# tkortz/opencv

Hardware: AMD Instinct MI355X
Metric: tracked frames/sec, 1080p×128-object TBD loop @ 1/2/4/8 MI355X (higher is better)
Workload: dtype u8; 1 GPU; TBD loop 1920x1080 x 128 objects (BASELINE configs[2]), frames [5, 2577) of a 2577-frame sequence per GPU; levels=3, win=21, gftt=256/box, q 0.01, minDist 3, every 5, tracker_bounds=reference, parallelism=replicas x1 (one sequence per GPU), api=tbdk_tbd_run (native frame loop, look-ahead)

## Files before the change

### opencv_amd/csrc/klt_lk_multi.hip

```cpp
#include <type_traits>

#include "lk_device.hpp"

namespace tbdk {

namespace {

using namespace lkdev;

__device__ __forceinline__ uint32_t scan64(uint32_t v)
{
    v += (uint32_t)__builtin_amdgcn_update_dpp(0, (int)v, 0x111, 0xF, 0xF, true);
    v += (uint32_t)__builtin_amdgcn_update_dpp(0, (int)v, 0x112, 0xF, 0xF, true);
    v += (uint32_t)__builtin_amdgcn_update_dpp(0, (int)v, 0x114, 0xF, 0xF, true);
    v += (uint32_t)__builtin_amdgcn_update_dpp(0, (int)v, 0x118, 0xF, 0xF, true);
    v += (uint32_t)__builtin_amdgcn_update_dpp(0, (int)v, 0x142, 0xA, 0xF, false);
    v += (uint32_t)__builtin_amdgcn_update_dpp(0, (int)v, 0x143, 0xC, 0xF, false);
    return v;
}

template <int M>
__device__ __forceinline__ void scan64_n(uint32_t (&v)[M])
{
#define TBDK_SCAN_STEP(ctrl, rmask, bc)                                                                    \
    _Pragma("unroll") for (int m = 0; m < M; ++m) v[m] +=                                                  \
        (uint32_t)__builtin_amdgcn_update_dpp(0, (int)v[m], ctrl, rmask, 0xF, bc);
    TBDK_SCAN_STEP(0x111, 0xF, true)
    TBDK_SCAN_STEP(0x112, 0xF, true)
    TBDK_SCAN_STEP(0x114, 0xF, true)
    TBDK_SCAN_STEP(0x118, 0xF, true)
    TBDK_SCAN_STEP(0x142, 0xA, false)
    TBDK_SCAN_STEP(0x143, 0xC, false)
#undef TBDK_SCAN_STEP
}

__device__ __forceinline__ uint32_t seg_total(uint32_t scanned, int e4, int s4)
{
    return (uint32_t)__builtin_amdgcn_ds_bpermute(e4, (int)scanned) -
           (uint32_t)__builtin_amdgcn_ds_bpermute(s4, (int)scanned);
}

template <int N, int FB = 26>
__device__ __forceinline__ void seg_sum_exact(const int (&v)[N], int e4, int s4, float (&out)[N], bool* split = nullptr)
{
    static_assert(N >= 1 && N <= 3, "three 11-bit fields per packed scan");
    static_assert(FB <= 26, "hi parts are v >> 26");
    bool big = false;
#pragma unroll
    for (int k = 0; k < N; ++k) big |= (uint32_t)v[k] + (1u << FB) >= (2u << FB);
    const bool slow = __builtin_amdgcn_ballot_w64(big) != 0;
    if (split) *split = slow;
    if (!slow) {
        uint32_t sv[N];
#pragma unroll
        for (int k = 0; k < N; ++k) sv[k] = (uint32_t)v[k];
        scan64_n(sv);
#pragma unroll
        for (int k = 0; k < N; ++k) out[k] = (float)(int)seg_total(sv[k], e4, s4);
        return;
    }
    uint32_t sc[N + 1];
    sc[N] = 0;
#pragma unroll
    for (int k = 0; k < N; ++k) {
        sc[k] = (uint32_t)v[k] & 0x3FFFFFFu;
        sc[N] += (uint32_t)(v[k] >> 26) << (11 * k);
    }
    scan64_n(sc);
    int h = (int)seg_total(sc[N], e4, s4);
#pragma unroll
    for (int k = 0; k < N; ++k) {
        const int hk = k + 1 < N ? (int)((uint32_t)h << 21) >> 21 : h;
        h = (h - hk) >> 11;
        const uint32_t l = seg_total(sc[k], e4, s4);
        out[k] = (float)((double)hk * 67108864.0 + (double)l);
    }
}

__device__ __forceinline__ int seg_sum_small(int v, int e4, int s4)
{
    return (int)seg_total(scan64((uint32_t)v), e4, s4);
}

__device__ __forceinline__ int bilin_c(uint32_t p0, uint32_t p1, uint32_t w0, uint32_t w1, int c)
{
    int t;
    asm("v_dot2_i32_i16 %0, %1, %2, %3" : "=v"(t) : "v"(p1), "v"(w1), "v"(c));
    return sdot2(p0, w0, t);
}

template <int SH>
__device__ __forceinline__ uint32_t pack_shr(int t0, int t1)
{
    uint32_t d = (uint32_t)(t0 >> SH);
    asm("v_ashrrev_i32_sdwa %0, %2, %1 dst_sel:WORD_1 dst_unused:UNUSED_PRESERVE src0_sel:DWORD src1_sel:DWORD"
        : "+v"(d)
        : "v"(t1), "i"(SH));
    return d;
}
__device__ __forceinline__ uint32_t pack_diff(int t0, int t1) { return pack_shr<9>(t0, t1); }

__device__ __forceinline__ bool any_lane(bool p) { return __builtin_amdgcn_ballot_w64(p) != 0; }


}

#ifndef TBDK_LK_IPACK
#define TBDK_LK_IPACK 1
#endif
#ifndef TBDK_LK_IPACK_FLY
#define TBDK_LK_IPACK_FLY 0
#endif

#ifdef TBDK_LK_TRACE
__device__ unsigned long long* g_lk_trace;
__device__ unsigned int g_lk_trace_cap;
static unsigned g_lk_trace_next;
#endif

template <int WW, int WH, bool FLY, bool DENSE = false>
__global__ __launch_bounds__(64) void lk_multi_kernel(LkArgs a)
{
    constexpr bool BACK = false;
    const LkBack bk{};
#include "klt_lk_multi_body.inc"
}

template <int WW, int WH>
__global__ __launch_bounds__(64) void lk_multi_back_kernel(LkArgs a, LkBack bk)
{
    constexpr bool BACK = true, FLY = true, DENSE = false;
#include "klt_lk_multi_body.inc"
}

#define TBDK_MULTI_WINDOWS(X) X(7) X(9) X(11) X(13) X(15) X(17) X(19) X(21) X(23) X(25) X(27) X(29) X(31)

bool lk_multi_supported(int win_w, int win_h)
{
    if (win_w != win_h) return false;
    switch (win_w) {
#define TBDK_CASE(W) case W:
        TBDK_MULTI_WINDOWS(TBDK_CASE)
#undef TBDK_CASE
        return true;
    default:
        return false;
    }
}

hipError_t launch_lk_multi(const LkArgs& a, bool fly, hipStream_t s)
{
    if (!lk_multi_supported(a.win_w, a.win_h)) return hipErrorNotSupported;
    const int per_wg = 64 / a.win_w;
    const dim3 grid((a.n + per_wg - 1) / per_wg), block(64);
#ifdef TBDK_LK_TRACE
    LkArgs at = a;
    at.trace_base = g_lk_trace_next;
    g_lk_trace_next += grid.x;
    const LkArgs& la = at;
#else
    const LkArgs& la = a;
#endif
    switch (a.win_w) {
#define TBDK_CASE(W)                                                                    \
    case W:                                                                             \
        if (fly) hipLaunchKernelGGL((lk_multi_kernel<W, W, true>), grid, block, 0, s, la);  \
        else hipLaunchKernelGGL((lk_multi_kernel<W, W, false>), grid, block, 0, s, la); \
        break;
        TBDK_MULTI_WINDOWS(TBDK_CASE)
#undef TBDK_CASE
    default:
        return hipErrorNotSupported;
    }
    return hipGetLastError();
}

hipError_t launch_lk_multi_back(const LkArgs& a, const LkBack& b, hipStream_t s)
{
    if (!lk_multi_supported(a.win_w, a.win_h)) return hipErrorNotSupported;
    const int per_wg = 64 / a.win_w;
    const dim3 grid((a.n + per_wg - 1) / per_wg), block(64);
#ifdef TBDK_LK_TRACE
    LkArgs at = a;
    at.trace_base = g_lk_trace_next;
    g_lk_trace_next += grid.x;
    const LkArgs& la = at;
#else
    const LkArgs& la = a;
#endif
    switch (a.win_w) {
#define TBDK_CASE(W)                                                              \
    case W:                                                                       \
        hipLaunchKernelGGL((lk_multi_back_kernel<W, W>), grid, block, 0, s, la, b); \
        break;
        TBDK_MULTI_WINDOWS(TBDK_CASE)
#undef TBDK_CASE
    default:
        return hipErrorNotSupported;
    }
    return hipGetLastError();
}

hipError_t launch_lk_multi_dense(const LkArgs& a, hipStream_t s)
{
    if (!lk_multi_supported(a.win_w, a.win_h)) return hipErrorNotSupported;
    const int per_wg = 64 / a.win_w;
    const dim3 grid((a.n + per_wg - 1) / per_wg), block(64);
    switch (a.win_w) {
#define TBDK_CASE(W)                                                                          \
    case W:                                                                                   \
        hipLaunchKernelGGL((lk_multi_kernel<W, W, false, true>), grid, block, 0, s, a);       \
        break;
        TBDK_MULTI_WINDOWS(TBDK_CASE)
#undef TBDK_CASE
    default:
        return hipErrorNotSupported;
    }
    return hipGetLastError();
}

}

#ifdef TBDK_LK_TRACE
extern "C" int tbdk_probe_lk_trace(void* buf, unsigned cap)
{
    unsigned long long* p = static_cast<unsigned long long*>(buf);
    cap /= 16;
    if (hipDeviceSynchronize() != hipSuccess ||
        hipMemcpyToSymbol(HIP_SYMBOL(tbdk::g_lk_trace), &p, sizeof(p)) != hipSuccess ||
        hipMemcpyToSymbol(HIP_SYMBOL(tbdk::g_lk_trace_cap), &cap, sizeof(cap)) != hipSuccess)
        return -2;
    tbdk::g_lk_trace_next = 0;
    return 0;
}
extern "C" int tbdk_probe_lk_trace_count(unsigned* n)
{
    *n = tbdk::g_lk_trace_next;
    return 0;
}
#endif
```

### opencv_amd/csrc/klt_lk_multi_body.inc

```
    static_assert(!DENSE || (!FLY && TBDK_LK_IPACK == 1), "dense mode: the planes instance's packed I pairs");
    static_assert(!BACK || (FLY && !DENSE), "backward mode: the Scharr-on-the-fly instance");
    constexpr int P = 64 / WW;
    constexpr int NP = (WH + 1) / 2;
    constexpr int IM = FLY ? TBDK_LK_IPACK_FLY : TBDK_LK_IPACK;
    constexpr bool IPACK = IM == 1, ILIN = IM == 2;
    constexpr bool kSoloOk = P >= 2 && !ILIN;
    const int lane = threadIdx.x & 63;
    const int k = lane == 0 ? P : (lane - 1) / WW;
    const int x = k < P ? lane - 1 - k * WW : 0;
    const int wave = xcd_swizzle(blockIdx.x, gridDim.x) + (threadIdx.x >> 6);
#ifdef TBDK_LK_TRACE
    const unsigned long long tr_t0 = __builtin_amdgcn_s_memrealtime();
#endif
    int i = -1;
    float p0x = 0.f, p0y = 0.f;
    float o0x = 0.f, o0y = 0.f;
    int fst = 0;
    if constexpr (DENSE) {
        i = k < P && wave * P + k < a.n ? wave * P + k : -1;
    } else {
        const int kk = wave * P + k;
        if (k < P && kk < a.n) {
            if (!a.seg_counts) {
                i = kk;
                p0x = a.prev_pts[2 * i];
                p0y = a.prev_pts[2 * i + 1];
                if constexpr (BACK) {
                    o0x = p0x;
                    o0y = p0y;
                    p0x = a.next_pts[2 * i];
                    p0y = a.next_pts[2 * i + 1];
                    fst = a.status[i];
                }
            } else {
                const int seg = kk / a.seg_stride, j = kk - seg * a.seg_stride;
                const int s = a.seg_ninl > 0 ? (int)a.seg_inl[seg] : a.seg_list ? a.seg_list[seg] : seg;
                const int cand = s * a.seg_stride + j;
                const int cnt = a.seg_counts[s];
                const float cx = a.prev_pts[2 * cand], cy = a.prev_pts[2 * cand + 1];
                float nx = 0.f, ny = 0.f;
                int cs = 0;
                if constexpr (BACK) {
                    nx = a.next_pts[2 * cand];
                    ny = a.next_pts[2 * cand + 1];
                    cs = a.status[cand];
                }
                if (j < cnt) {
                    i = cand;
                    p0x = cx;
                    p0y = cy;
                    if constexpr (BACK) {
                        o0x = cx;
                        o0y = cy;
                        p0x = nx;
                        p0y = ny;
                        fst = cs;
                    }
                }
            }
        }
    }
    if constexpr (BACK) {
        if (i >= 0 && !fst) {
            if (x == 0) {
                if (bk.back_pts) {
                    bk.back_pts[2 * i] = o0x;
                    bk.back_pts[2 * i + 1] = o0y;
                }
                if (bk.fb_err) bk.fb_err[i] = __builtin_inff();
            }
            i = -1;
        }
    }
    const bool valid = i >= 0;
    if (!any_lane(valid)) return;
#ifdef TBDK_LK_TRACE
    int tr_steps = 0, tr_reloads = 0;
    unsigned tr_gsplit = 0;
    auto tr_stamp = [&](int idx) {
        const unsigned r = a.trace_base + (unsigned)wave;
        const unsigned d = (unsigned)(__builtin_amdgcn_s_memrealtime() - tr_t0);
        if (lane == 0 && r < g_lk_trace_cap) reinterpret_cast<unsigned*>(g_lk_trace + 16ull * r + 6)[idx] = d;
    };
#else
    auto tr_stamp = [](int) {};
#endif
#ifdef TBDK_LK_TRACE
    asm volatile("s_waitcnt vmcnt(0)" ::: "memory");
    tr_stamp(13);
#endif
    const int e4 = 4 * (k * WW + WW), s4 = 4 * (k * WW);
    const int rnd9 = __builtin_amdgcn_readfirstlane(1 << (W_BITS1 - 5 - 1));
    const int rnd14 = __builtin_amdgcn_readfirstlane(1 << (W_BITS1 - 1));

    const float FLT_SCALE = 1.f / (1 << 20);
    const float halfx = (WW - 1) * 0.5f, halfy = (WH - 1) * 0.5f;
    const int gy = DENSE && valid ? i / a.dense_w : 0, gx = DENSE && valid ? i - gy * a.dense_w : 0;
    if constexpr (DENSE) {
        p0x = (float)gx;
        p0y = (float)gy;
    }
    float outx = 0.f, outy = 0.f;
    if (((BACK ? 0 : a.flags) & TBDK_OPTFLOW_USE_INITIAL_FLOW) && valid) {
        outx = a.next_pts[2 * i];
        outy = a.next_pts[2 * i + 1];
    }
    int status = 1, nit = 0;
#if defined(TBDK_LK_PROBE_RELOADS) && TBDK_LK_PROBE_RELOADS == 2
    int nrl = 0;
#endif
    float errv = 0.f;

    for (int level = a.max_level; level >= 0; --level) {
        const LkLevel L = a.lv[level];
        tr_stamp(4 * level);
        const float sc = (float)(1. / (1 << level));
        float prevx = p0x * sc, prevy = p0y * sc;
        float nextx, nexty;
        if (level == a.max_level) {
            if ((BACK ? 0 : a.flags) & TBDK_OPTFLOW_USE_INITIAL_FLOW) {
                nextx = outx * sc;
                nexty = outy * sc;
            } else {
                nextx = prevx;
                nexty = prevy;
            }
        } else {
            nextx = outx * 2.f;
            nexty = outy * 2.f;
        }
        outx = nextx;
        outy = nexty;

        prevx -= halfx;
        prevy -= halfy;
        const int ipx = (int)floorf(prevx), ipy = (int)floorf(prevy);
        bool act = valid;
        if (ipx < -WW || ipx >= L.w || ipy < -WH || ipy >= L.h) {
            if (level == 0) {
                status = 0;
                errv = 0.f;
            }
            act = false;
        }
        if (!any_lane(act)) continue;
        uint32_t w0, w1;
        bilinear_weights(prevx - ipx, prevy - ipy, w0, w1);

        uint32_t jp[WH + 1];
        const int hp = L.h + 2 * L.ipad;
        const __amdgpu_buffer_rsrc_t rI = make_rsrc(L.I, rsrc_bytes(L.ipitch, hp, L.ipad ? 256 : 0));
        const __amdgpu_buffer_rsrc_t rD = make_rsrc(L.D, rsrc_bytes(L.dpitch, L.h + 2 * L.dpad, 256));
        const __amdgpu_buffer_rsrc_t rJ = make_rsrc(L.J, rsrc_bytes(L.jpitch, L.h + 2 * L.jpad, L.jpad ? 256 : 0));
        auto load_j = [&](bool on, int jx0, int jy0) {
            if (L.jpad == 0 &&
                any_lane(on && (jx0 + x < 0 || jx0 + x + 1 >= L.w || jy0 < 0 || jy0 + WH >= L.h))) {
#pragma unroll
                for (int r = 0; r <= WH; ++r)
                    jp[r] = on ? load_pair_refl(rJ, L.jpitch, L.w, L.h, jy0 + r, jx0 + x) : 0u;
                return;
            }
            const uint32_t joff = on ? (uint32_t)(jy0 + L.jpad) * (uint32_t)L.jpitch + (uint32_t)(jx0 + x + L.jpad) : 0u;
#pragma unroll
            for (int r = 0; r <= WH; ++r) jp[r] = load_pair_u8_ua(rJ, joff, (int)((uint32_t)r * (uint32_t)L.jpitch));
        };

        nextx -= halfx;
        nexty -= halfy;
        int pinx = (int)floorf(nextx), piny = (int)floorf(nexty);

        uint32_t ipk[IPACK ? NP : 1];
        int ic[IM == 0 ? WH : 1];
        int cgx = 0, cgy = 0;
        uint32_t gxk[NP], gyk[NP];
        float A11, A12, A22;
        {
            int acc[3] = {0, 0, 0};
            auto pair_step = [&](int q, uint32_t ip0, uint32_t ip1, uint32_t ip2, uint32_t dx0, uint32_t dx1,
                                 uint32_t dx2, uint32_t dy0, uint32_t dy1, uint32_t dy2, uint32_t dw0, uint32_t dw1,
                                 uint32_t dw2, uint32_t dw3) {
                const int r = 2 * q;
                const bool two = r + 1 < WH;
                uint32_t ipq = 0;
                if constexpr (IPACK || ILIN) {
                    const int i0 = bilin_s<0>(ip0, ip1, w0, w1, rnd9);
                    const int i1 = two ? bilin_s<0>(ip1, ip2, w0, w1, rnd9) : 0;
                    ipq = pack_shr<W_BITS1 - 5>(i0, i1);
                    if constexpr (IPACK) ipk[q] = ipq;
                } else {
                    ic[r] = rnd9 - (bilin_s<W_BITS1 - 5>(ip0, ip1, w0, w1, rnd9) << 9);
                    if (two) ic[r + 1] = rnd9 - (bilin_s<W_BITS1 - 5>(ip1, ip2, w0, w1, rnd9) << 9);
                }
                const int x0 = bilin_s<0>(dx0, dx1, dw0, dw1, rnd14);
                const int x1 = two ? bilin_s<0>(dx1, dx2, dw2, dw3, rnd14) : 0;
                const int y0 = bilin_s<0>(dy0, dy1, dw0, dw1, rnd14);
                const int y1 = two ? bilin_s<0>(dy1, dy2, dw2, dw3, rnd14) : 0;
                gxk[q] = pack_shr<W_BITS1>(x0, x1);
                gyk[q] = pack_shr<W_BITS1>(y0, y1);
                if constexpr (ILIN) {
                    cgx = sdot2(ipq, gxk[q], cgx);
                    cgy = sdot2(ipq, gyk[q], cgy);
                }
                acc[0] = sdot2(gxk[q], gxk[q], acc[0]);
                acc[1] = sdot2(gxk[q], gyk[q], acc[1]);
                acc[2] = sdot2(gyk[q], gyk[q], acc[2]);
            };
            if constexpr (FLY) {
                const uint32_t ioff =
                    act ? (uint32_t)(ipy - 1 + L.ipad) * (uint32_t)L.ipitch + (uint32_t)(ipx + x - 1 + L.ipad) : 0u;
                uint32_t u[WH + 3];
                if (L.ipad == 0 &&
                    any_lane(act && (ipx + x - 1 < 0 || ipx + x + 2 >= L.w || ipy - 1 < 0 || ipy + WH + 1 >= L.h))) {
#pragma unroll
                    for (int r = 0; r < WH + 3; ++r)
                        u[r] = act ? load4_refl(rI, L.ipitch, L.w, L.h, ipy - 1 + r, ipx + x - 1) : 0u;
                } else {
#pragma unroll
                    for (int r = 0; r < WH + 3; ++r)
                        u[r] = __builtin_amdgcn_raw_buffer_load_b32(rI, ioff, (int)((uint32_t)r * (uint32_t)L.ipitch), 0);
                }
#ifdef TBDK_LK_TRACE
                asm volatile("s_waitcnt vmcnt(0)" ::: "memory");
                if (level == a.max_level) tr_stamp(14);
#endif
                const uint32_t cm = ((unsigned)(ipx + x) < (unsigned)L.w ? 0x0000FFFFu : 0u) |
                                    ((unsigned)(ipx + x + 1) < (unsigned)L.w ? 0xFFFF0000u : 0u);
                const int rlo = min(max(-ipy, 0), 32), rhi = min(max(L.h - ipy, 0), 32);
                const uint32_t vm = (uint32_t)(((1ull << rhi) - 1ull) & ~((1ull << rlo) - 1ull));
                const uint32_t wd0 = w0 & cm, wd1 = w1 & cm;
                auto rowbit = [&](int r) { return (uint32_t)((int)(vm << (31 - r)) >> 31); };
                auto src = [&](int j, uint32_t& mid, uint32_t& hd, uint32_t& sm) {
                    const u16x2 lo = as_u16x2(__builtin_amdgcn_perm(0u, u[j], 0x0C010C00u));
                    const u16x2 hi = as_u16x2(__builtin_amdgcn_perm(0u, u[j], 0x0C030C02u));
                    mid = __builtin_amdgcn_perm(0u, u[j], 0x0C020C01u);
                    hd = as_u32(hi - lo);
                    sm = as_u32((lo + hi) * (unsigned short)3 + as_u16x2(mid) * (unsigned short)10);
                };
                auto drow = [&](uint32_t hda, uint32_t hdb, uint32_t hdc, uint32_t sma, uint32_t smc, uint32_t& dx,
                                uint32_t& dy) {
                    dx = as_u32((as_u16x2(hda) + as_u16x2(hdc)) * (unsigned short)3 + as_u16x2(hdb) * (unsigned short)10);
                    dy = as_u32(as_u16x2(smc) - as_u16x2(sma));
                };
                uint32_t m0, h0, s0, m1, h1, s1, m2, h2, s2;
                src(0, m0, h0, s0);
                src(1, m1, h1, s1);
                src(2, m2, h2, s2);
                uint32_t dxa, dya;
                drow(h0, h1, h2, s0, s2, dxa, dya);
                uint32_t ipa = m1;
                uint32_t ra = rowbit(0);
#pragma unroll
                for (int q = 0; q < NP; ++q) {
                    const int r = 2 * q;
                    m0 = m1; h0 = h1; s0 = s1;
                    m1 = m2; h1 = h2; s1 = s2;
                    src(r + 3, m2, h2, s2);
                    uint32_t dxb, dyb, dxc = 0, dyc = 0, ipc = 0;
                    drow(h0, h1, h2, s0, s2, dxb, dyb);
                    const uint32_t ipb = m1;
                    const uint32_t rb = rowbit(r + 1);
                    uint32_t rc = 0;
                    if (r + 1 < WH) {
                        m0 = m1; h0 = h1; s0 = s1;
                        m1 = m2; h1 = h2; s1 = s2;
                        src(r + 4, m2, h2, s2);
                        drow(h0, h1, h2, s0, s2, dxc, dyc);
                        ipc = m1;
                        rc = rowbit(r + 2);
                    }
                    pair_step(q, ipa, ipb, ipc, dxa, dxb, dxc, dya, dyb, dyc, wd0 & ra, wd1 & rb, wd0 & rb, wd1 & rc);
                    ipa = ipc;
                    dxa = dxc;
                    dya = dyc;
                    ra = rc;
                }
            } else if constexpr (DENSE) {
                const int msk = (1 << level) - 1;
                const int64_t cbase = act ? (int64_t)(((gy & msk) << level) | (gx & msk)) * L.cstride +
                                                (int64_t)ipy * L.cpitch + ipx + x
                                          : -(int64_t)(WH / 2) * L.cpitch - WW / 2;
                const uint2* cw = L.C + cbase;
#pragma unroll
                for (int q = 0; q < NP; ++q) {
                    const int r = 2 * q;
                    const uint2 e0 = cw[(int64_t)r * L.cpitch];
                    const uint2 e1 = r + 1 < WH ? cw[(int64_t)(r + 1) * L.cpitch] : make_uint2(0u, 0u);
                    ipk[q] = __builtin_amdgcn_perm(e1.x, e0.x, 0x05040100u);
                    gxk[q] = __builtin_amdgcn_perm(e1.x, e0.x, 0x07060302u);
                    gyk[q] = __builtin_amdgcn_perm(e1.y, e0.y, 0x05040100u);
                    acc[0] = sdot2(gxk[q], gxk[q], acc[0]);
                    acc[1] = sdot2(gxk[q], gyk[q], acc[1]);
                    acc[2] = sdot2(gyk[q], gyk[q], acc[2]);
                }
            } else {
                uint32_t ip[WH + 1], dxp[WH + 1], dyp[WH + 1];
                const uint32_t ioff = act ? (uint32_t)((ipy + L.ipad) * L.ipitch + ipx + x + L.ipad) : 0u;
                const uint32_t doff = act ? (uint32_t)((ipy + L.dpad) * L.dpitch + (ipx + x + L.dpad) * 4) : 0u;
#pragma unroll
                for (int r = 0; r <= WH; ++r) {
                    ip[r] = load_pair_u8_ua(rI, ioff, r * L.ipitch);
                    const uint32_t d0 = __builtin_amdgcn_raw_buffer_load_b32(rD, doff, r * L.dpitch, 0);
                    const uint32_t d1 = __builtin_amdgcn_raw_buffer_load_b32(rD, doff + 4, r * L.dpitch, 0);
                    dxp[r] = __builtin_amdgcn_perm(d1, d0, 0x05040100u);
                    dyp[r] = __builtin_amdgcn_perm(d1, d0, 0x07060302u);
                }
#pragma unroll
                for (int q = 0; q < NP; ++q) {
                    const int r = 2 * q;
                    const int r2 = r + 2 <= WH ? r + 2 : WH;
                    pair_step(q, ip[r], ip[r + 1], ip[r2], dxp[r], dxp[r + 1], dxp[r2], dyp[r], dyp[r + 1], dyp[r2],
                              w0, w1, w0, w1);
                }
            }
            if constexpr (IPACK) {
#pragma unroll
                for (int q = 0; q < NP; ++q) asm volatile("" : "+v"(ipk[q]));
            }
#ifdef TBDK_LK_TRACE
            __builtin_amdgcn_sched_barrier(0);
            if (level == a.max_level) tr_stamp(15);
            __builtin_amdgcn_sched_barrier(0);
#endif
            if (k >= P) acc[0] = acc[1] = acc[2] = 0;
            float s[3];
#ifdef TBDK_LK_TRACE
            bool tr_split = false;
            seg_sum_exact<3>(acc, e4, s4, s, &tr_split);
            tr_gsplit |= tr_split ? 1u << level : 0u;
#else
            seg_sum_exact<3>(acc, e4, s4, s);
#endif
            tr_stamp(4 * level + 1);
            {
                const bool jin = act && !(pinx < -WW || pinx >= L.w || piny < -WH || piny >= L.h);
                load_j(jin, pinx, piny);
#ifdef TBDK_LK_TRACE
                asm volatile("s_waitcnt vmcnt(0)" ::: "memory");
#endif
                tr_stamp(4 * level + 2);
            }
            A11 = s[0] * FLT_SCALE;
            A12 = s[1] * FLT_SCALE;
            A22 = s[2] * FLT_SCALE;
        }
        float D = A11 * A22 - A12 * A12;
        const float minEig =
            (A22 + A11 - sqrtf((A11 - A22) * (A11 - A22) + 4.f * A12 * A12)) / (float)(2 * WW * WH);
        if (act && ((BACK ? 0 : a.flags) & TBDK_OPTFLOW_LK_GET_MIN_EIGENVALS)) errv = minEig;
        if (act && (minEig < a.min_eig || D < 1.19209290e-07F )) {
            if (level == 0) status = 0;
            act = false;
        }
        D = 1.f / D;

        float pdx = 0.f, pdy = 0.f;
        auto solo_steps = [&](int ks, int j) {
            constexpr int NPG = (NP + P - 1) / P;
            constexpr int RG = 2 * NPG;
            const int sl = 1 + ks * WW;
            const int src = k < P ? 4 * (sl + x) : 0;
            const int g = k < P ? k : 0;
            uint32_t gx2[NPG], gy2[NPG], ip2[IPACK ? NPG : 1];
            int ic2[IM == 0 ? RG : 1];
#pragma unroll
            for (int t = 0; t < NPG; ++t) gx2[t] = gy2[t] = 0u;
            if constexpr (IPACK) {
#pragma unroll
                for (int t = 0; t < NPG; ++t) ip2[t] = 0u;
            }
            if constexpr (IM == 0) {
#pragma unroll
                for (int t = 0; t < RG; ++t) ic2[t] = 0;
            }
#pragma unroll
            for (int q = 0; q < NP; ++q) {
                const uint32_t tx = (uint32_t)__builtin_amdgcn_ds_bpermute(src, (int)gxk[q]);
                const uint32_t ty = (uint32_t)__builtin_amdgcn_ds_bpermute(src, (int)gyk[q]);
                gx2[q % NPG] = g == q / NPG ? tx : gx2[q % NPG];
                gy2[q % NPG] = g == q / NPG ? ty : gy2[q % NPG];
                if constexpr (IPACK) {
                    const uint32_t ti = (uint32_t)__builtin_amdgcn_ds_bpermute(src, (int)ipk[q]);
                    ip2[q % NPG] = g == q / NPG ? ti : ip2[q % NPG];
                }
            }
            if constexpr (IM == 0) {
#pragma unroll
                for (int r = 0; r < WH; ++r) {
                    const int ti = __builtin_amdgcn_ds_bpermute(src, ic[r]);
                    ic2[r % RG] = g == r / RG ? ti : ic2[r % RG];
                }
            }
            if (k >= P) {
#pragma unroll
                for (int t = 0; t < NPG; ++t) gx2[t] = gy2[t] = 0u;
            }
            auto bc = [&](float v) { return __int_as_float(__builtin_amdgcn_readlane(__float_as_int(v), sl)); };
            float snx = bc(nextx), sny = bc(nexty), sox = bc(outx), soy = bc(outy), spdx = bc(pdx), spdy = bc(pdy);
            const float sA11 = bc(A11), sA12 = bc(A12), sA22 = bc(A22), sD = bc(D);
            const int rbase = g * RG;
            uint32_t jp2[RG + 1];
            auto load_j2 = [&](int jx0, int jy0) {
                const uint32_t joff = (uint32_t)((jy0 + rbase + L.jpad) * L.jpitch + jx0 + x + L.jpad);
#pragma unroll
                for (int r = 0; r <= RG; ++r) jp2[r] = load_pair_u8_ua(rJ, joff, r * L.jpitch);
            };
            int qx = INT_MIN, qy = 0, snit = 0;
            bool sout = false;
            for (; j < a.max_count; ++j) {
                const int inx = (int)floorf(snx), iny = (int)floorf(sny);
                if (inx < -WW || inx >= L.w || iny < -WH || iny >= L.h) {
                    sout = true;
                    break;
                }
                ++snit;
#ifdef TBDK_LK_TRACE
                ++tr_steps;
#endif
                if (inx != qx || iny != qy) {
#ifdef TBDK_LK_TRACE
                    ++tr_reloads;
#endif
                    load_j2(inx, iny);
                    qx = inx;
                    qy = iny;
                }
                uint32_t v0, v1;
                bilinear_weights(snx - inx, sny - iny, v0, v1);
                int b[2] = {0, 0};
#pragma unroll
                for (int t = 0; t < NPG; ++t) {
                    uint32_t d;
                    if constexpr (IPACK) {
                        const uint32_t jv = pack_diff(bilin_s<0>(jp2[2 * t], jp2[2 * t + 1], v0, v1, rnd9),
                                                      bilin_s<0>(jp2[2 * t + 1], jp2[2 * t + 2], v0, v1, rnd9));
                        d = as_u32(as_s16x2(jv) - as_s16x2(ip2[t]));
                    } else {
                        d = pack_diff(bilin_c(jp2[2 * t], jp2[2 * t + 1], v0, v1, ic2[2 * t]),
                                      bilin_c(jp2[2 * t + 1], jp2[2 * t + 2], v0, v1, ic2[2 * t + 1]));
                    }
                    b[0] = sdot2(d, gx2[t], b[0]);
                    b[1] = sdot2(d, gy2[t], b[1]);
                }
                float fb[2];
                seg_sum_exact<2, 25>(b, 4 * (P * WW), 0, fb);
                const float fb1 = fb[0] * FLT_SCALE;
                const float fb2 = fb[1] * FLT_SCALE;
                const float ddx = (sA12 * fb2 - sA22 * fb1) * sD;
                const float ddy = (sA12 * fb1 - sA11 * fb2) * sD;
                snx += ddx;
                sny += ddy;
                sox = snx + halfx;
                soy = sny + halfy;
                if ((double)ddx * ddx + (double)ddy * ddy <= a.eps2) break;
                if (j > 0 && (double)fabsf(ddx + spdx) < 0.01 && (double)fabsf(ddy + spdy) < 0.01) {
                    sox -= ddx * 0.5f;
                    soy -= ddy * 0.5f;
                    break;
                }
                spdx = ddx;
                spdy = ddy;
            }
            if (k == ks) {
                outx = sox;
                outy = soy;
#ifdef TBDK_LK_PROBE_ITERS_LV
                nit += snit << (8 * level);
#else
                nit += snit;
#endif
                if (sout && level == 0) status = 0;
            }
            act = false;
        };
        for (int j = 0; j < a.max_count; ++j) {
            if (!any_lane(act)) break;
#ifdef TBDK_LK_TRACE
            ++tr_steps;
#endif
            if constexpr (kSoloOk) {
                if (a.solo_min > 0 && j >= a.solo_min && L.jpad > 0) {
                    const uint64_t heads = __builtin_amdgcn_ballot_w64(act && x == 0 && k < P);
                    if (__builtin_popcountll(heads) == 1) {
                        solo_steps((__builtin_ctzll(heads) - 1) / WW, j);
                        break;
                    }
                }
            }
            const int inx = (int)floorf(nextx), iny = (int)floorf(nexty);
            if (act && (inx < -WW || inx >= L.w || iny < -WH || iny >= L.h)) {
                if (level == 0) status = 0;
                act = false;
            }
#ifdef TBDK_LK_PROBE_ITERS_LV
            nit += act ? 1 << (8 * level) : 0;
#else
            nit += act ? 1 : 0;
#endif
            const bool moved = act && (inx != pinx || iny != piny);
#ifdef TBDK_LK_PROBE_RELOADS
#if TBDK_LK_PROBE_RELOADS == 2
            nrl += any_lane(moved) ? 1 : 0;
#endif
            if (TBDK_LK_PROBE_RELOADS == 1 || (TBDK_LK_PROBE_RELOADS != 3 && any_lane(moved))) {
#else
            if (any_lane(moved)) {
#endif
#ifdef TBDK_LK_TRACE
                ++tr_reloads;
#endif
                load_j(act, inx, iny);
                pinx = inx;
                piny = iny;
            }
            bilinear_weights(nextx - inx, nexty - iny, w0, w1);
            int b[2] = {0, 0};
#pragma unroll
            for (int q = 0; q < NP; ++q) {
                const int r = 2 * q;
                uint32_t d;
                if constexpr (ILIN) {
                    d = r + 1 < WH ? pack_diff(bilin_s<0>(jp[r], jp[r + 1], w0, w1, rnd9),
                                               bilin_s<0>(jp[r + 1], jp[r + 2], w0, w1, rnd9))
                                   : pack_diff(bilin_s<0>(jp[r], jp[r + 1], w0, w1, rnd9), 0);
                } else if constexpr (IPACK) {
                    const uint32_t jv = r + 1 < WH ? pack_diff(bilin_s<0>(jp[r], jp[r + 1], w0, w1, rnd9),
                                                               bilin_s<0>(jp[r + 1], jp[r + 2], w0, w1, rnd9))
                                                   : pack_diff(bilin_s<0>(jp[r], jp[r + 1], w0, w1, rnd9), 0);
                    d = as_u32(as_s16x2(jv) - as_s16x2(ipk[q]));
                } else {
                    d = r + 1 < WH ? pack_diff(bilin_c(jp[r], jp[r + 1], w0, w1, ic[r]),
                                               bilin_c(jp[r + 1], jp[r + 2], w0, w1, ic[r + 1]))
                                   : pack_diff(bilin_c(jp[r], jp[r + 1], w0, w1, ic[r]), 0);
                }
                const uint32_t gx = gxk[q], gy = gyk[q];
                b[0] = sdot2(d, gx, b[0]);
                b[1] = sdot2(d, gy, b[1]);
#ifdef TBDK_LK_NEWTON_SB
                if (q % TBDK_LK_NEWTON_SB == TBDK_LK_NEWTON_SB - 1) __builtin_amdgcn_sched_barrier(0);
#endif
            }
            if constexpr (ILIN) {
                b[0] -= cgx;
                b[1] -= cgy;
            }
            if (k >= P) b[0] = b[1] = 0;
            float fb[2];
            seg_sum_exact<2>(b, e4, s4, fb);
            const float fb1 = fb[0] * FLT_SCALE;
            const float fb2 = fb[1] * FLT_SCALE;
            const float ddx = (A12 * fb2 - A22 * fb1) * D;
            const float ddy = (A12 * fb1 - A11 * fb2) * D;
            if (act) {
                nextx += ddx;
                nexty += ddy;
                outx = nextx + halfx;
                outy = nexty + halfy;
                if ((double)ddx * ddx + (double)ddy * ddy <= a.eps2) {
                    act = false;
                } else if (j > 0 && (double)fabsf(ddx + pdx) < 0.01 && (double)fabsf(ddy + pdy) < 0.01) {
                    outx -= ddx * 0.5f;
                    outy -= ddy * 0.5f;
                    act = false;
                }
                pdx = ddx;
                pdy = ddy;
            }
        }

        tr_stamp(4 * level + 3);
        if (!BACK && level == 0 && a.err && ((BACK ? 0 : a.flags) & TBDK_OPTFLOW_LK_GET_MIN_EIGENVALS) == 0) {
            bool want = valid && status;
            const float npx = outx - halfx, npy = outy - halfy;
            const int inx = (int)floorf(npx), iny = (int)floorf(npy);
            if (want && (inx < -WW || inx >= L.w || iny < -WH || iny >= L.h)) {
                status = 0;
                want = false;
            }
            if (any_lane(want)) {
                uint32_t ipr[ILIN ? NP : 1];
                if constexpr (ILIN) {
                    uint32_t iw0, iw1;
                    bilinear_weights(prevx - ipx, prevy - ipy, iw0, iw1);
                    const bool irefl = L.ipad == 0 && any_lane(want && (ipx + x < 0 || ipx + x + 1 >= L.w ||
                                                                        ipy < 0 || ipy + WH >= L.h));
                    const uint32_t ioff =
                        want ? (uint32_t)(ipy + L.ipad) * (uint32_t)L.ipitch + (uint32_t)(ipx + x + L.ipad) : 0u;
                    auto irow = [&](int r) -> uint32_t {
                        if (irefl) return want ? load_pair_refl(rI, L.ipitch, L.w, L.h, ipy + r, ipx + x) : 0u;
                        return load_pair_u8_ua(rI, ioff, (int)((uint32_t)r * (uint32_t)L.ipitch));
                    };
                    uint32_t ra = irow(0);
#pragma unroll
                    for (int q = 0; q < NP; ++q) {
                        const int r = 2 * q;
                        const uint32_t rb = irow(r + 1);
                        const uint32_t rc = r + 2 <= WH ? irow(r + 2) : 0u;
                        ipr[q] = pack_shr<W_BITS1 - 5>(bilin_s<0>(ra, rb, iw0, iw1, rnd9),
                                                        r + 1 < WH ? bilin_s<0>(rb, rc, iw0, iw1, rnd9) : 0);
                        asm volatile("" : "+v"(ipr[q]));
                        ra = rc;
                    }
                }
                bilinear_weights(npx - inx, npy - iny, w0, w1);
                load_j(want, inx, iny);
                int e = 0;
#pragma unroll
                for (int q = 0; q < NP; ++q) {
                    const int r = 2 * q;
                    int d0;
                    if constexpr (ILIN)
                        d0 = (bilin_s<0>(jp[r], jp[r + 1], w0, w1, rnd9) >> 9) - (int)(int16_t)(ipr[q] & 0xFFFFu);
                    else if constexpr (IPACK)
                        d0 = (bilin_s<0>(jp[r], jp[r + 1], w0, w1, rnd9) >> 9) - (int)(int16_t)(ipk[q] & 0xFFFFu);
                    else
                        d0 = bilin_c(jp[r], jp[r + 1], w0, w1, ic[r]) >> 9;
                    e += d0 < 0 ? -d0 : d0;
                    if (r + 1 < WH) {
                        int d1;
                        if constexpr (ILIN)
                            d1 = (bilin_s<0>(jp[r + 1], jp[r + 2], w0, w1, rnd9) >> 9) - (int)(int16_t)(ipr[q] >> 16);
                        else if constexpr (IPACK)
                            d1 = (bilin_s<0>(jp[r + 1], jp[r + 2], w0, w1, rnd9) >> 9) - (int)(int16_t)(ipk[q] >> 16);
                        else
                            d1 = bilin_c(jp[r + 1], jp[r + 2], w0, w1, ic[r + 1]) >> 9;
                        e += d1 < 0 ? -d1 : d1;
                    }
                }
                if (k >= P) e = 0;
                const float errval = (float)seg_sum_small(e, e4, s4);
                if (want) errv = errval * 1.f / (float)(32 * WW * WH);
                tr_stamp(12);
            }
        }
    }

#ifdef TBDK_LK_TRACE
    {
        int mx = 0;
#pragma unroll
        for (int q = 0; q < P; ++q) mx = max(mx, __builtin_amdgcn_readlane(valid ? nit : 0, 1 + q * WW));
        const unsigned long long tr_t1 = __builtin_amdgcn_s_memrealtime();
        const unsigned hw = __builtin_amdgcn_s_getreg((31 << 11) | 4);
        const unsigned xcc = __builtin_amdgcn_s_getreg((15 << 11) | 20);
        if (lane == 0) {
            const unsigned r = a.trace_base + (unsigned)wave;
            if (r < g_lk_trace_cap) {
                unsigned long long* o = g_lk_trace + 16ull * r;
                o[0] = tr_t0;
                o[1] = tr_t1;
                o[2] = hw | ((unsigned long long)xcc << 32);
                o[3] = ((unsigned long long)(unsigned)a.n << 32) | (unsigned)wave;
                o[4] = a.seg_ninl > 0 ? (1ull << 48) | ((unsigned long long)a.seg_ninl << 16) | a.seg_inl[0]
                                      : (unsigned long long)(uintptr_t)(a.seg_list ? (const void*)a.seg_list
                                                                                   : (const void*)a.prev_pts);
                o[5] = (unsigned)tr_steps | ((unsigned long long)(unsigned)tr_reloads << 16) |
                       ((unsigned long long)(unsigned)mx << 32) | ((unsigned long long)tr_gsplit << 48);
            }
        }
    }
#endif
    if constexpr (BACK) {
        if (valid && x == 0) {
            const float dx = fabsf(o0x - outx), dy = fabsf(o0y - outy);
            const float d = fmaxf(dx, dy);
            if (bk.back_pts) {
                bk.back_pts[2 * i] = outx;
                bk.back_pts[2 * i + 1] = outy;
            }
            if (bk.fb_err) bk.fb_err[i] = status ? d : __builtin_inff();
            if (!(status && d < bk.thr)) a.status[i] = 0;
        }
        return;
    }
    if (DENSE && valid && x == 0) {
        *reinterpret_cast<float2*>(reinterpret_cast<uint8_t*>(a.flow) + (size_t)gy * a.flow_pitch + 8 * (size_t)gx) =
            make_float2(outx - (float)gx, outy - (float)gy);
        if (a.dstatus) a.dstatus[(size_t)gy * a.dstatus_pitch + gx] = (uint8_t)status;
        return;
    }
    if (valid && x == 0) {
        a.next_pts[2 * i] = outx;
        a.next_pts[2 * i + 1] = outy;
        a.status[i] = (uint8_t)status;
        if (a.err) a.err[i] = errv;
#if defined(TBDK_LK_PROBE_RELOADS) && TBDK_LK_PROBE_RELOADS == 2
        nit += 1000 * nrl;
#endif
        if (a.iters) a.iters[i] = nit;
    }
```

### opencv_amd/csrc/lk_device.hpp

```cpp
#pragma once
#include "tbdk_internal.hpp"

namespace tbdk {
namespace lkdev {

constexpr int W_BITS = 14, W_BITS1 = 14;

typedef short s16x2 __attribute__((ext_vector_type(2)));
typedef unsigned short u16x2 __attribute__((ext_vector_type(2)));

__device__ __forceinline__ u16x2 as_u16x2(uint32_t v) { return __builtin_bit_cast(u16x2, v); }
__device__ __forceinline__ uint32_t as_u32(u16x2 v) { return __builtin_bit_cast(uint32_t, v); }
__device__ __forceinline__ s16x2 as_s16x2(uint32_t v) { return __builtin_bit_cast(s16x2, v); }
__device__ __forceinline__ uint32_t as_u32(s16x2 v) { return __builtin_bit_cast(uint32_t, v); }

__device__ __forceinline__ int sdot2(uint32_t a, uint32_t b, int c)
{
    return __builtin_amdgcn_sdot2(__builtin_bit_cast(s16x2, a), __builtin_bit_cast(s16x2, b), c, false);
}

__device__ __forceinline__ int bilin(uint32_t p0, uint32_t p1, uint32_t w0, uint32_t w1, int shift)
{
    return sdot2(p0, w0, sdot2(p1, w1, 1 << (shift - 1))) >> shift;
}

template <int SHIFT>
__device__ __forceinline__ int bilin_s(uint32_t p0, uint32_t p1, uint32_t w0, uint32_t w1, int round_sgpr)
{
    int t;
    asm("v_dot2_i32_i16 %0, %1, %2, %3" : "=v"(t) : "v"(p1), "v"(w1), "s"(round_sgpr));
    return sdot2(p0, w0, t) >> SHIFT;
}

__device__ __forceinline__ void bilinear_weights(float fa, float fb, uint32_t& w0, uint32_t& w1)
{
    constexpr float kMagic = 12582912.f;
    const float ga = 1.f - fa, gb = 1.f - fb;
    const uint32_t b00 = __float_as_uint(__builtin_fmaf(ga * gb, (float)(1 << W_BITS), kMagic));
    const uint32_t b01 = __float_as_uint(__builtin_fmaf(fa * gb, (float)(1 << W_BITS), kMagic));
    const uint32_t b10 = __float_as_uint(__builtin_fmaf(ga * fb, (float)(1 << W_BITS), kMagic));
    const uint32_t b11 = (uint32_t)(1 << W_BITS) - (b00 + b01 + b10);
    w0 = __builtin_amdgcn_perm(b01, b00, 0x05040100u);
    w1 = __builtin_amdgcn_perm(b11, b10, 0x05040100u);
}

__device__ __forceinline__ __amdgpu_buffer_rsrc_t make_rsrc(const void* base, uint32_t bytes)
{
    return __builtin_amdgcn_make_buffer_rsrc(const_cast<void*>(base), (short)0, (int)bytes, 0x00020000);
}

__device__ __forceinline__ uint32_t rsrc_bytes(int pitch, int rows, int room = 0)
{
    return (uint32_t)pitch * (uint32_t)rows + (uint32_t)room;
}

__device__ __forceinline__ uint32_t load_pair_u8(__amdgpu_buffer_rsrc_t rs, uint32_t aligned, int soff, uint32_t sel)
{
    const uint32_t lo = __builtin_amdgcn_raw_buffer_load_b32(rs, aligned, soff, 0);
    const uint32_t hi = __builtin_amdgcn_raw_buffer_load_b32(rs, aligned + 4, soff, 0);
    return __builtin_amdgcn_perm(hi, lo, sel);
}

__device__ __forceinline__ uint32_t load_pair_u8_ua(__amdgpu_buffer_rsrc_t rs, uint32_t off, int soff)
{
    const uint32_t v = __builtin_amdgcn_raw_buffer_load_b32(rs, off, soff, 0);
    return __builtin_amdgcn_perm(v, v, 0x0C010C00u);
}


__device__ __forceinline__ int refl101(int c, int n)
{
    c = c < 0 ? -c : c;
    return c >= n ? 2 * (n - 1) - c : c;
}

__device__ __forceinline__ uint32_t load4_refl(__amdgpu_buffer_rsrc_t rs, int pitch, int w, int h, int row, int col)
{
    const uint32_t yo = (uint32_t)refl101(row, h) * (uint32_t)pitch;
    uint32_t v = 0;
#pragma unroll
    for (int k = 0; k < 4; ++k)
        v |= (uint32_t)__builtin_amdgcn_raw_buffer_load_b8(rs, yo + (uint32_t)refl101(col + k, w), 0, 0) << (8 * k);
    return v;
}

__device__ __forceinline__ uint32_t load_pair_refl(__amdgpu_buffer_rsrc_t rs, int pitch, int w, int h, int row, int col)
{
    const uint32_t yo = (uint32_t)refl101(row, h) * (uint32_t)pitch;
    const uint32_t a = __builtin_amdgcn_raw_buffer_load_b8(rs, yo + (uint32_t)refl101(col, w), 0, 0);
    const uint32_t b = __builtin_amdgcn_raw_buffer_load_b8(rs, yo + (uint32_t)refl101(col + 1, w), 0, 0);
    return a | (b << 16);
}

__device__ __forceinline__ uint32_t pair_sel(uint32_t off)
{
    return 0x0C000C00u | ((off & 3u) + (((off & 3u) + 1u) << 16));
}

__device__ __forceinline__ bool out_of_level(float fx, float fy, int ix, int iy, int ww, int wh, int w, int h)
{
    return fx != fx || fy != fy || ix < -ww || ix >= w || iy < -wh || iy >= h;
}

}
}
```

Measured before the change: 6186 frames/s.

## Make LK Newton loop wave-uniform with ballot masks and cheaper stop tests

Restructures the per-feature Lucas-Kanade iteration to track activity as a wave-level ballot mask instead of per-lane branches. The double-precision convergence test becomes a float test with safety bounds, falling back to the exact double check only when a value is ambiguous. Gradient rows skip the per-row mask multiply when no active lane touches the image edge, and padding lanes get zero weights instead of being zeroed after accumulation. The first dot-product in each chain drops its accumulator input. The solo-feature handoff now runs after the loop exits. This adds a second specialised row path, which may increase code size and register pressure, and the oscillation test changes from strict < 0.01 in double to <= 0.01f.

```diff
diff --git a/opencv_amd/csrc/klt_lk_multi.hip b/opencv_amd/csrc/klt_lk_multi.hip
--- a/opencv_amd/csrc/klt_lk_multi.hip
+++ b/opencv_amd/csrc/klt_lk_multi.hip
@@ -1,6 +1,7 @@
 #include <type_traits>
 
 #include "lk_device.hpp"
+#include "lk_stop.hpp"
 
 namespace tbdk {
 
diff --git a/opencv_amd/csrc/klt_lk_multi_body.inc b/opencv_amd/csrc/klt_lk_multi_body.inc
--- a/opencv_amd/csrc/klt_lk_multi_body.inc
+++ b/opencv_amd/csrc/klt_lk_multi_body.inc
@@ -8,7 +8,7 @@
     const int lane = threadIdx.x & 63;
     const int k = lane == 0 ? P : (lane - 1) / WW;
     const int x = k < P ? lane - 1 - k * WW : 0;
-    const int wave = xcd_swizzle(blockIdx.x, gridDim.x) + (threadIdx.x >> 6);
+    const int wave = xcd_swizzle(blockIdx.x, gridDim.x);
 #ifdef TBDK_LK_TRACE
     const unsigned long long tr_t0 = __builtin_amdgcn_s_memrealtime();
 #endif
@@ -92,6 +92,9 @@
     const int e4 = 4 * (k * WW + WW), s4 = 4 * (k * WW);
     const int rnd9 = __builtin_amdgcn_readfirstlane(1 << (W_BITS1 - 5 - 1));
     const int rnd14 = __builtin_amdgcn_readfirstlane(1 << (W_BITS1 - 1));
+    const lkstop::EpsBounds eb0 = lkstop::eps_bounds(a.eps2);
+    const lkstop::EpsBounds eb = {__int_as_float(__builtin_amdgcn_readfirstlane(__float_as_int(eb0.lo))),
+                                  __int_as_float(__builtin_amdgcn_readfirstlane(__float_as_int(eb0.hi)))};
 
     const float FLT_SCALE = 1.f / (1 << 20);
     const float halfx = (WW - 1) * 0.5f, halfy = (WH - 1) * 0.5f;
@@ -146,6 +149,9 @@
         if (!any_lane(act)) continue;
         uint32_t w0, w1;
         bilinear_weights(prevx - ipx, prevy - ipy, w0, w1);
+        if constexpr (!DENSE) {
+            if (k >= P) w0 = w1 = 0u;
+        }
 
         uint32_t jp[WH + 1];
         const int hp = L.h + 2 * L.ipad;
@@ -223,6 +229,7 @@
                 asm volatile("s_waitcnt vmcnt(0)" ::: "memory");
                 if (level == a.max_level) tr_stamp(14);
 #endif
+                const bool edge = any_lane(act && (ipx + x < 0 || ipx + x + 1 >= L.w || ipy < 0 || ipy + WH >= L.h));
                 const uint32_t cm = ((unsigned)(ipx + x) < (unsigned)L.w ? 0x0000FFFFu : 0u) |
                                     ((unsigned)(ipx + x + 1) < (unsigned)L.w ? 0xFFFF0000u : 0u);
                 const int rlo = min(max(-ipy, 0), 32), rhi = min(max(L.h - ipy, 0), 32);
@@ -241,39 +248,53 @@
                     dx = as_u32((as_u16x2(hda) + as_u16x2(hdc)) * (unsigned short)3 + as_u16x2(hdb) * (unsigned short)10);
                     dy = as_u32(as_u16x2(smc) - as_u16x2(sma));
                 };
+                auto rows = [&](auto masked) {
+                constexpr bool MASKED = decltype(masked)::value;
+                auto srca = [&](int j, uint32_t& mid, uint32_t& hd, uint32_t& sm) {
+                    if constexpr (MASKED) asm volatile("; masked row" : "+v"(u[j]));
+                    else asm volatile("; plain row" : "+v"(u[j]));
+                    src(j, mid, hd, sm);
+                };
                 uint32_t m0, h0, s0, m1, h1, s1, m2, h2, s2;
-                src(0, m0, h0, s0);
-                src(1, m1, h1, s1);
-                src(2, m2, h2, s2);
+                srca(0, m0, h0, s0);
+                srca(1, m1, h1, s1);
+                srca(2, m2, h2, s2);
                 uint32_t dxa, dya;
                 drow(h0, h1, h2, s0, s2, dxa, dya);
                 uint32_t ipa = m1;
-                uint32_t ra = rowbit(0);
+                uint32_t ra = MASKED ? rowbit(0) : 0u;
 #pragma unroll
                 for (int q = 0; q < NP; ++q) {
                     const int r = 2 * q;
                     m0 = m1; h0 = h1; s0 = s1;
                     m1 = m2; h1 = h2; s1 = s2;
-                    src(r + 3, m2, h2, s2);
+                    srca(r + 3, m2, h2, s2);
                     uint32_t dxb, dyb, dxc = 0, dyc = 0, ipc = 0;
                     drow(h0, h1, h2, s0, s2, dxb, dyb);
                     const uint32_t ipb = m1;
-                    const uint32_t rb = rowbit(r + 1);
+                    const uint32_t rb = MASKED ? rowbit(r + 1) : 0u;
                     uint32_t rc = 0;
                     if (r + 1 < WH) {
                         m0 = m1; h0 = h1; s0 = s1;
                         m1 = m2; h1 = h2; s1 = s2;
-                        src(r + 4, m2, h2, s2);
+                        srca(r + 4, m2, h2, s2);
                         drow(h0, h1, h2, s0, s2, dxc, dyc);
                         ipc = m1;
-                        rc = rowbit(r + 2);
+                        if constexpr (MASKED) rc = rowbit(r + 2);
                     }
-                    pair_step(q, ipa, ipb, ipc, dxa, dxb, dxc, dya, dyb, dyc, wd0 & ra, wd1 & rb, wd0 & rb, wd1 & rc);
+                    if constexpr (MASKED)
+                        pair_step(q, ipa, ipb, ipc, dxa, dxb, dxc, dya, dyb, dyc, wd0 & ra, wd1 & rb, wd0 & rb, wd1 & rc);
+                    else
+                        pair_step(q, ipa, ipb, ipc, dxa, dxb, dxc, dya, dyb, dyc, w0, w1, w0, w1);
                     ipa = ipc;
                     dxa = dxc;
                     dya = dyc;
                     ra = rc;
                 }
+                };
+                if (edge) rows(std::true_type{});
+                else rows(std::false_type{});
+                __builtin_amdgcn_sched_barrier(0);
             } else if constexpr (DENSE) {
                 const int msk = (1 << level) - 1;
                 const int64_t cbase = act ? (int64_t)(((gy & msk) << level) | (gx & msk)) * L.cstride +
@@ -321,7 +342,9 @@
             if (level == a.max_level) tr_stamp(15);
             __builtin_amdgcn_sched_barrier(0);
 #endif
-            if (k >= P) acc[0] = acc[1] = acc[2] = 0;
+            if constexpr (DENSE) {
+                if (k >= P) acc[0] = acc[1] = acc[2] = 0;
+            }
             float s[3];
 #ifdef TBDK_LK_TRACE
             bool tr_split = false;
@@ -353,7 +376,7 @@
         }
         D = 1.f / D;
 
-        float pdx = 0.f, pdy = 0.f;
+        float pdx = __builtin_inff(), pdy = __builtin_inff();
         auto solo_steps = [&](int ks, int j) {
             constexpr int NPG = (NP + P - 1) / P;
             constexpr int RG = 2 * NPG;
@@ -438,8 +461,8 @@
                         d = pack_diff(bilin_c(jp2[2 * t], jp2[2 * t + 1], v0, v1, ic2[2 * t]),
                                       bilin_c(jp2[2 * t + 1], jp2[2 * t + 2], v0, v1, ic2[2 * t + 1]));
                     }
-                    b[0] = sdot2(d, gx2[t], b[0]);
-                    b[1] = sdot2(d, gy2[t], b[1]);
+                    b[0] = t ? sdot2(d, gx2[t], b[0]) : sdot2_first(d, gx2[t]);
+                    b[1] = t ? sdot2(d, gy2[t], b[1]) : sdot2_first(d, gy2[t]);
                 }
                 float fb[2];
                 seg_sum_exact<2, 25>(b, 4 * (P * WW), 0, fb);
@@ -451,8 +474,17 @@
                 sny += ddy;
                 sox = snx + halfx;
                 soy = sny + halfy;
-                if ((double)ddx * ddx + (double)ddy * ddy <= a.eps2) break;
-                if (j > 0 && (double)fabsf(ddx + spdx) < 0.01 && (double)fabsf(ddy + spdy) < 0.01) {
+                const float q = lkstop::eps_q(ddx, ddy);
+                const uint64_t belowm = __builtin_amdgcn_ballot_w64(lkstop::eps_below(q, eb));
+                const uint64_t abovem = __builtin_amdgcn_ballot_w64(lkstop::eps_above(q, eb));
+                bool reached = belowm != 0;
+                if ((belowm | abovem) == 0) {
+                    asm volatile("" ::: "memory");
+                    reached = __builtin_amdgcn_ballot_w64(lkstop::eps_exact(ddx, ddy, a.eps2)) != 0;
+                }
+                if (reached) break;
+                if ((__builtin_amdgcn_ballot_w64(lkstop::osc_small(ddx + spdx)) &
+                     __builtin_amdgcn_ballot_w64(lkstop::osc_small(ddy + spdy))) != 0) {
                     sox -= ddx * 0.5f;
                     soy -= ddy * 0.5f;
                     break;
@@ -472,43 +504,39 @@
             }
             act = false;
         };
-        for (int j = 0; j < a.max_count; ++j) {
-            if (!any_lane(act)) break;
+        const auto bal = [](bool p) { return __builtin_amdgcn_ballot_w64(p); };
+        uint64_t actm = bal(act);
+        const uint64_t headm = bal(x == 0 && k < P);
+        int solo_ks = -1, solo_j = 0;
+        for (int j = 0; j < a.max_count && actm != 0;) {
 #ifdef TBDK_LK_TRACE
             ++tr_steps;
 #endif
-            if constexpr (kSoloOk) {
-                if (a.solo_min > 0 && j >= a.solo_min && L.jpad > 0) {
-                    const uint64_t heads = __builtin_amdgcn_ballot_w64(act && x == 0 && k < P);
-                    if (__builtin_popcountll(heads) == 1) {
-                        solo_steps((__builtin_ctzll(heads) - 1) / WW, j);
-                        break;
-                    }
-                }
-            }
             const int inx = (int)floorf(nextx), iny = (int)floorf(nexty);
-            if (act && (inx < -WW || inx >= L.w || iny < -WH || iny >= L.h)) {
-                if (level == 0) status = 0;
-                act = false;
-            }
+            {
+                const uint64_t oobm = bal(inx < -WW) | bal(inx >= L.w) | bal(iny < -WH) | bal(iny >= L.h);
+                status = __builtin_amdgcn_inverse_ballot_w64(level == 0 ? actm & oobm : 0ull) ? 0 : status;
+                actm &= ~oobm;
+            }
+            const bool on = __builtin_amdgcn_inverse_ballot_w64(actm);
 #ifdef TBDK_LK_PROBE_ITERS_LV
-            nit += act ? 1 << (8 * level) : 0;
+            nit += on ? 1 << (8 * level) : 0;
 #else
-            nit += act ? 1 : 0;
-#endif
-            const bool moved = act && (inx != pinx || iny != piny);
+            nit += on ? 1 : 0;
+#endif
+            const uint64_t movedm = (bal(inx != pinx) | bal(iny != piny)) & actm;
 #ifdef TBDK_LK_PROBE_RELOADS
 #if TBDK_LK_PROBE_RELOADS == 2
-            nrl += any_lane(moved) ? 1 : 0;
-#endif
-            if (TBDK_LK_PROBE_RELOADS == 1 || (TBDK_LK_PROBE_RELOADS != 3 && any_lane(moved))) {
+            nrl += movedm != 0 ? 1 : 0;
+#endif
+            if (TBDK_LK_PROBE_RELOADS == 1 || (TBDK_LK_PROBE_RELOADS != 3 && movedm != 0)) {
 #else
-            if (any_lane(moved)) {
+            if (movedm != 0) {
 #endif
 #ifdef TBDK_LK_TRACE
                 ++tr_reloads;
 #endif
-                load_j(act, inx, iny);
+                load_j(on, inx, iny);
                 pinx = inx;
                 piny = iny;
             }
@@ -532,9 +560,8 @@
                                                bilin_c(jp[r + 1], jp[r + 2], w0, w1, ic[r + 1]))
                                    : pack_diff(bilin_c(jp[r], jp[r + 1], w0, w1, ic[r]), 0);
                 }
-                const uint32_t gx = gxk[q], gy = gyk[q];
-                b[0] = sdot2(d, gx, b[0]);
-                b[1] = sdot2(d, gy, b[1]);
+                b[0] = q ? sdot2(d, gxk[q], b[0]) : sdot2_first(d, gxk[q]);
+                b[1] = q ? sdot2(d, gyk[q], b[1]) : sdot2_first(d, gyk[q]);
 #ifdef TBDK_LK_NEWTON_SB
                 if (q % TBDK_LK_NEWTON_SB == TBDK_LK_NEWTON_SB - 1) __builtin_amdgcn_sched_barrier(0);
 #endif
@@ -543,27 +570,54 @@
                 b[0] -= cgx;
                 b[1] -= cgy;
             }
-            if (k >= P) b[0] = b[1] = 0;
+            if constexpr (DENSE) {
+                if (k >= P) b[0] = b[1] = 0;
+            }
             float fb[2];
             seg_sum_exact<2>(b, e4, s4, fb);
             const float fb1 = fb[0] * FLT_SCALE;
             const float fb2 = fb[1] * FLT_SCALE;
             const float ddx = (A12 * fb2 - A22 * fb1) * D;
             const float ddy = (A12 * fb1 - A11 * fb2) * D;
-            if (act) {
-                nextx += ddx;
-                nexty += ddy;
-                outx = nextx + halfx;
-                outy = nexty + halfy;
-                if ((double)ddx * ddx + (double)ddy * ddy <= a.eps2) {
-                    act = false;
-                } else if (j > 0 && (double)fabsf(ddx + pdx) < 0.01 && (double)fabsf(ddy + pdy) < 0.01) {
-                    outx -= ddx * 0.5f;
-                    outy -= ddy * 0.5f;
-                    act = false;
-                }
-                pdx = ddx;
-                pdy = ddy;
+            const float q = lkstop::eps_q(ddx, ddy);
+            const uint64_t belowm = bal(lkstop::eps_below(q, eb)), abovem = bal(lkstop::eps_above(q, eb));
+            uint64_t reachm = belowm;
+            if ((~(belowm | abovem) & actm) != 0) {
+                asm volatile("" ::: "memory");
+                reachm = bal(lkstop::eps_exact(ddx, ddy, a.eps2));
+            }
+            const uint64_t oscm = bal(lkstop::osc_small(ddx + pdx)) & bal(lkstop::osc_small(ddy + pdy));
+            const float nx = nextx + ddx, ny = nexty + ddy;
+            float ox = nx + halfx, oy = ny + halfy;
+            if (__builtin_amdgcn_inverse_ballot_w64(oscm & ~reachm)) {
+                ox -= ddx * 0.5f;
+                oy -= ddy * 0.5f;
+            }
+            nextx = on ? nx : nextx;
+            nexty = on ? ny : nexty;
+            outx = on ? ox : outx;
+            outy = on ? oy : outy;
+            actm &= ~(reachm | oscm);
+            pdx = ddx;
+            pdy = ddy;
+            ++j;
+            if constexpr (kSoloOk) {
+                if (a.solo_min > 0 && j >= a.solo_min && L.jpad > 0) {
+                    const uint64_t heads = actm & headm;
+                    if (__builtin_popcountll(heads) == 1) {
+                        solo_ks = (__builtin_ctzll(heads) - 1) / WW;
+                        solo_j = j;
+                        break;
+                    }
+                }
+            }
+        }
+        if constexpr (kSoloOk) {
+            if (solo_ks >= 0 && solo_j < a.max_count) {
+#ifdef TBDK_LK_TRACE
+                ++tr_steps;
+#endif
+                solo_steps(solo_ks, solo_j);
             }
         }
 
diff --git a/opencv_amd/csrc/lk_device.hpp b/opencv_amd/csrc/lk_device.hpp
--- a/opencv_amd/csrc/lk_device.hpp
+++ b/opencv_amd/csrc/lk_device.hpp
@@ -17,6 +17,13 @@
 __device__ __forceinline__ int sdot2(uint32_t a, uint32_t b, int c)
 {
     return __builtin_amdgcn_sdot2(__builtin_bit_cast(s16x2, a), __builtin_bit_cast(s16x2, b), c, false);
+}
+
+__device__ __forceinline__ int sdot2_first(uint32_t a, uint32_t b)
+{
+    int t;
+    asm("v_dot2_i32_i16 %0, %1, %2, 0" : "=v"(t) : "v"(a), "v"(b));
+    return t;
 }
 
 __device__ __forceinline__ int bilin(uint32_t p0, uint32_t p1, uint32_t w0, uint32_t w1, int shift)
diff --git a/opencv_amd/csrc/lk_stop.hpp b/opencv_amd/csrc/lk_stop.hpp
--- /dev/null
+++ b/opencv_amd/csrc/lk_stop.hpp
@@ -0,0 +1,45 @@
+#pragma once
+
+#if defined(__HIPCC__)
+#define TBDK_LK_HD __host__ __device__ inline
+#else
+#define TBDK_LK_HD inline
+#endif
+
+namespace tbdk {
+namespace lkstop {
+
+TBDK_LK_HD bool eps_exact(float ddx, float ddy, double eps2) { return (double)ddx * ddx + (double)ddy * ddy <= eps2; }
+TBDK_LK_HD bool osc_exact(float s) { return (double)__builtin_fabsf(s) < 0.01; }
+
+TBDK_LK_HD bool osc_small(float s) { return __builtin_fabsf(s) <= 0.01f; }
+
+struct EpsBounds {
+    float lo, hi;
+};
+
+TBDK_LK_HD EpsBounds eps_bounds(double eps2)
+{
+    EpsBounds b;
+    b.lo = -__builtin_inff();
+    b.hi = __builtin_inff();
+    if (eps2 >= 0x1p-100 && eps2 <= 0x1p100) {
+        b.lo = (float)(eps2 * (1.0 - 0x1p-19));
+        b.hi = (float)(eps2 * (1.0 + 0x1p-19));
+    }
+    return b;
+}
+
+TBDK_LK_HD float eps_q(float ddx, float ddy) { return ddx * ddx + ddy * ddy; }
+TBDK_LK_HD bool eps_below(float q, EpsBounds b) { return q < b.lo; }
+TBDK_LK_HD bool eps_above(float q, EpsBounds b) { return q > b.hi; }
+TBDK_LK_HD bool eps_ambiguous(float q, EpsBounds b) { return !eps_below(q, b) && !eps_above(q, b); }
+
+TBDK_LK_HD bool eps_reached(float ddx, float ddy, double eps2, EpsBounds b)
+{
+    const float q = eps_q(ddx, ddy);
+    return eps_ambiguous(q, b) ? eps_exact(ddx, ddy, eps2) : eps_below(q, b);
+}
+
+}
+}
```

Result: faster. 6323 frames/s (median of 6 runs) (+2.2%).
